# YihangChen-ee/CNC

Measured on AMD Instinct MI355X. Metric: ray-samples/s/GPU (16Lx2^19xF8 grid), higher is better.
Workload: dtype f32; 1 GPU; configs[1]: 800x800 rays/GPU marched (step 5e-3) through a 128^3 ball occupancy, every sample encoded fwd (sign bit plane) + bwd (STE mask) on the binarised 16Lx2^19xF8 hash grid; rays_per_gpu=640000, chunk=1048576, table_rows=6120776, n_features=8, levels=16

## Files before the change

cnc_amd/_lib.py:

```python
from __future__ import annotations

import ctypes as C
import os

import torch

_HERE = os.path.dirname(os.path.abspath(__file__))
LIB_PATH = os.path.join(_HERE, "libcnc_hip.so")
_lib = None

_vp, _u32, _i32, _i64, _f32 = C.c_void_p, C.c_uint32, C.c_int32, C.c_int64, C.c_float


class RaySegments(C.Structure):
    _fields_ = [("vals", _vp), ("chunk_starts", _vp), ("chunk_cnts", _vp), ("ray_indices", _vp),
                ("is_left", _vp), ("is_right", _vp), ("is_valid", _vp)]


class PdfRows(C.Structure):
    _fields_ = [("seg", RaySegments), ("n_rays", _i64), ("n_edges_per_ray", _i64), ("n_edges", _i64)]


class CtxWindow(C.Structure):
    _fields_ = [("pos", _vp * 16), ("cnt", _vp * 16), ("val", _vp * 16), ("p_at", _i64 * 17), ("v_at", _i64 * 17),
# ... 134 lines not shown
    "cnc_rows_scatter": [_vp, _vp, _vp, C.c_uint64, _u32, _vp],
    "cnc_table_adam": [_vp] + [C.c_double] * 6 + [_vp],
    "cnc_ray_window_positions": [_vp] * 10 + [_u32, _vp],
    "cnc_scatter_counted": [_vp, _vp, _vp, _vp, C.c_uint64, _vp],
    "cnc_ctx_compact": [_vp, _vp, _vp, _vp, C.c_uint64, _i32, _vp, _vp, _vp, _vp, _vp],
    "cnc_plane_ring_vertices": [_vp, C.c_uint64, _u32, _u32, C.c_uint64, _vp, _vp, _vp],
    "cnc_bernoulli_bits_partials": [C.c_uint64, _u32],
    "cnc_bernoulli_bits_forward": [_vp, _vp, _vp, C.c_uint64, _u32, _vp, _vp],
    "cnc_bernoulli_bits_backward": [_vp, _vp, _vp, _vp, C.c_uint64, _u32, _vp, _vp, _vp],
    "cnc_segment_weighted_sum_backward": [_vp, _vp, _vp, _vp, _u32, C.c_uint64, _u32, _i32, _vp, _vp],
    "cnc_segment_weighted_sum_gathered_backward": [_vp, _vp, _vp, _vp, _vp, _u32, C.c_uint64, _u32, _i32, _vp, _vp],
}

RESTYPES = {"cnc_grid_encode_backward_binned_workspace": C.c_uint64,
            "cnc_grid_encode_backward_overlapped_workspace": C.c_uint64, "cnc_bernoulli_bits_partials": C.c_uint32,
            "cnc_relu_backward_bias_partials": C.c_uint32, "cnc_occupancy_coarse_words": C.c_uint32}

CNC_FLAG_STE_BINARY = 1
CNC_FLAG_LEVELS_FINEST_FIRST = 2
CNC_FLAG_BIN_LANE_STORES = 4
CNC_FLAG_CELL_MERGE = 8
CNC_FLAG_CELL_CARRY = 16
CNC_FLAG_OWNER_XCD_PAIRS = 32
CNC_FIELD_SH_FP16 = 1
CNC_FIELD_MFMA_F16X3 = 2
CNC_FIELD_TWO_WAVES = 4
CNC_FIELD_WAVES4 = 8
CNC_PACK_TRANSPOSE = 1
CNC_PACK_ZERO_FIRST = 2
CNC_VOLREND_ACCUMULATE = 1
CNC_VOLREND_FINALIZE = 2
ABI_VERSION = 32


def lib() -> C.CDLL:
    global _lib
    if _lib is None:
        if not os.path.exists(LIB_PATH):
            raise RuntimeError(
                f"{LIB_PATH} not found: the HIP extension is required (no CPU fallback). "
                "Build it with `python -m cnc_amd.build`.")
        L = C.CDLL(LIB_PATH)
        for name, argtypes in SIGNATURES.items():
            fn = getattr(L, name)
            fn.argtypes = argtypes
            fn.restype = RESTYPES.get(name, C.c_int)
# ... 50 lines not shown
```

cnc_amd/backends/gridencoder_backend.py:

```python
from __future__ import annotations

import os

import torch

from .. import _lib
from .._lib import check, check_contiguous, check_cuda, ptr, stream

_FLOATING = (torch.float32, torch.float16, torch.float64)


def _check_floating(t, name):
    if t.dtype not in _FLOATING:
        raise RuntimeError(f"{name} must be a floating tensor")


def _check_int(t, name):
    if t.dtype != torch.int32:
        raise RuntimeError(f"{name} must be an int tensor")


def _require_f32(t, name):
    if t.dtype != torch.float32:
        raise RuntimeError(f"{name}: libcnc_hip builds the fp32 path only (got {t.dtype})")
# ... 100 lines not shown
                    ("offsets_list", offsets_list), ("resolutions_list", resolutions_list),
                    ("grad_embeddings", grad_embeddings)])
    _check_floating(grad, "grad")
    _check_floating(inputs, "inputs")
    _check_floating(embeddings, "embeddings")
    _check_int(offsets_list, "offsets_list")
    _check_int(resolutions_list, "resolutions_list")
    _check_floating(grad_embeddings, "grad_embeddings")
    for name, t in (("grad", grad), ("inputs", inputs), ("embeddings", embeddings),
                    ("grad_embeddings", grad_embeddings)):
        _require_f32(t, name)
    if n_features not in (1, 2, 4, 8, 16, 32):
        raise RuntimeError("GridEncoding: n_fearures must be 1, 2, 4, 8, 16 or 32.")
    if num_dim not in (1, 2, 3):
        raise RuntimeError("GridEncoding: num_dim must be 1, 2, 3.")
    if binary_vxl is not None:
        binary_vxl = binary_vxl.contiguous()
    if binned is not None and binned[0] > 0 and binary_vxl is None and min_level_id is None \
            and dy_dx is None and grad_inputs is None:
        n_binned, level_rows = int(binned[0]), int(binned[1])
        L = _lib.lib()
        nbytes = int(L.cnc_grid_encode_backward_binned_workspace(int(N), n_binned, level_rows))
        flags = (_lib.CNC_FLAG_STE_BINARY if ste_binary else 0) | (_lib.CNC_FLAG_BIN_LANE_STORES if _BIN_LANE_STORES else 0) \
            | (_lib.CNC_FLAG_OWNER_XCD_PAIRS if _OWNER_XCD_PAIRS else 0)
        if overlap_streams and _OVERLAP_ENABLED:
            cur = torch.cuda.current_stream(grad.device).cuda_stream
            nbytes = int(L.cnc_grid_encode_backward_overlapped_workspace(int(N), n_binned, level_rows))
            ws = _workspace(grad.device, nbytes, (cur, 0))
            rc = L.cnc_grid_encode_backward_overlapped(
                _plan(grad.device, cur), ptr(grad), ptr(inputs), ptr(embeddings), ptr(offsets_list), ptr(resolutions_list),
                ptr(grad_embeddings), int(N), int(num_dim), int(n_features), int(n_levels), flags, ptr(ste_clip_count),
                int(grad_ld), int(grad_col), n_binned, level_rows, ptr(ws),
                nbytes, stream(grad.device))
            check(rc, "grid_encode_backward_overlapped")
            return
        ws = _workspace(grad.device, nbytes, (torch.cuda.current_stream(grad.device).cuda_stream, 0))
        rc = L.cnc_grid_encode_backward_binned(
            ptr(grad), ptr(inputs), ptr(embeddings), ptr(offsets_list), ptr(resolutions_list),
            ptr(grad_embeddings), int(N), int(num_dim), int(n_features), int(n_levels), flags,
            ptr(ste_clip_count), int(grad_ld), int(grad_col), n_binned, level_rows, ptr(ws), nbytes,
            stream(grad.device))
        check(rc, "grid_encode_backward_binned")
        return
    rc = _lib.lib().cnc_grid_encode_backward(
        ptr(grad), ptr(inputs), ptr(embeddings), ptr(offsets_list), ptr(resolutions_list),
        ptr(grad_embeddings), int(N), int(num_dim), int(n_features), int(n_levels), int(Rb),
        ptr(dy_dx), ptr(grad_inputs), ptr(binary_vxl), ptr(min_level_id),
        (_lib.CNC_FLAG_STE_BINARY if ste_binary else 0)
        | (_lib.CNC_FLAG_LEVELS_FINEST_FIRST if interleave_levels else 0)
        | (_lib.CNC_FLAG_CELL_MERGE if cell_merge else 0)
        | (_lib.CNC_FLAG_CELL_CARRY if cell_merge and cell_carry else 0), ptr(ste_clip_count),
        ptr(_check_sat(occ_sat, binary_vxl)), *_vb(vertex_bits, binary_vxl, 0 if min_level_id is not None else n_levels),
        int(grad_ld), int(grad_col), stream(grad.device))
    check(rc, "grid_encode_backward")


_WORKSPACES = {}
_PLANS = {}
_OVERLAP_ENABLED = os.environ.get("CNC_BWD_OVERLAP", "1") != "0"
_BIN_LANE_STORES = os.environ.get("CNC_BWD_BIN_LANE_STORES", "0") == "1"
_OWNER_XCD_PAIRS = os.environ.get("CNC_BWD_OWNER_XCD_PAIRS", "0") == "1"


def _plan(device, caller_stream):
    import ctypes as C
    key = (device.type, device.index, caller_stream)
    h = _PLANS.get(key)
    if h is None:
        out = C.c_void_p()
        with torch.cuda.device(device):
            check(_lib.lib().cnc_backward_plan_create(C.byref(out)), "backward_plan_create")
        h = _PLANS[key] = out
    return h


def _workspace(device, nbytes, which=0):
    key = (device.type, device.index, which)
    ws = _WORKSPACES.get(key)
    if ws is None or ws.numel() < nbytes:
        ws = torch.empty(nbytes, dtype=torch.uint8, device=device)
        _WORKSPACES[key] = ws
    return ws


# ... 233 lines not shown
```

cnc_amd/csrc/common.hpp:

```cpp
#pragma once

#include <hip/hip_runtime.h>
#include <stdint.h>
#include <stdlib.h>

#include "cnc_hip.h"

namespace cnc {

constexpr int kWave = 64;

__host__ __device__ inline uint32_t div_up(uint32_t a, uint32_t b) { return (a + b - 1) / b; }

struct FeatLayout {
    uint32_t ld;
    uint32_t col;
    uint32_t finest_first = 0;
    uint32_t n_slots = 0;
    const uint32_t* vbits = nullptr;
    const int32_t*  vboff = nullptr;
    uint32_t        nt = 0;
};

__device__ __forceinline__ const uint32_t* vertex_plane(const FeatLayout& lay, uint32_t level)
{
    if (lay.vbits == nullptr) return nullptr;
    const int32_t w = lay.vboff[level];
    return w < 0 ? nullptr : lay.vbits + w;
}

__device__ __forceinline__ size_t feat_index(FeatLayout lay, uint32_t slot, uint32_t N, uint32_t b,
                                             uint32_t F)
{
    return lay.ld ? (size_t)b * lay.ld + lay.col + slot * F : ((size_t)slot * N + b) * F;
}

inline int launch_status()
{
    return hipGetLastError() == hipSuccess ? CNC_OK : CNC_ERR_LAUNCH;
}

template <uint32_t D>
__device__ __forceinline__ uint32_t grid_row(const uint32_t (&q)[D], uint32_t hashmap_size,
                                             uint32_t resolution)
{
    constexpr uint32_t primes[7] = {1u, 2654435761u, 805459861u, 3674653429u,
                                    2097192037u, 1434869437u, 2165219737u};
    uint32_t stride = 1, index = 0;
#pragma unroll
    for (uint32_t d = 0; d < D; d++) {
        if (stride <= hashmap_size) {
            index += q[d] * stride;
            stride *= resolution;
        }
    }
    if (stride > hashmap_size) {
        index = 0;
#pragma unroll
// ... 82 lines not shown
```

cnc_amd/csrc/grid_encode.hip:

```cpp
#include "common.hpp"
#include <cstdlib>

#include "encoder_common.hpp"

namespace cnc {

template <uint32_t D, uint32_t F, bool VXL, bool STE>
__global__ __launch_bounds__(256) void k_grid_encode_fwd(
    const float* __restrict__ inputs, const float* __restrict__ emb,
    const int32_t* __restrict__ offsets, const int32_t* __restrict__ resolutions,
    float* __restrict__ out, uint32_t N, uint32_t Rb, const uint8_t* __restrict__ vxl,
    const int32_t* __restrict__ min_level_id, const int32_t* __restrict__ sat, FeatLayout lay)
{
    constexpr uint32_t V = F < 4 ? F : 4;
    constexpr uint32_t G = F / V;
    constexpr uint32_t C = 1u << D;

    const uint32_t t = blockIdx.x * blockDim.x + threadIdx.x;
    const uint32_t b = t / G;
    const uint32_t h = t % G;
    if (b >= N) return;
    const uint32_t slot = blockIdx.y;
    const uint32_t level = slot + (min_level_id ? (uint32_t)min_level_id[b] : 0u);

// ... 615 lines not shown
    if (!cnt_loc(inputs + (size_t)b * 3, R, F, axis, q, loc)) return;
    const size_t   at = (size_t)grid_row<3>(q, hs, R) * F;
    const uint32_t half = loc / 2;
    const float gv = 1 / out_sum[half + ch];
    const bool  pos = (double)emb[at + ch] > 0.9;
    const float contrib = pos ? gv * grad[loc + ch * 2 + 0] : -gv * grad[loc + ch * 2 + 1];
    unsafeAtomicAdd(grad_emb + at + ch, contrib);
}

struct EncArgs {
    const float*   inputs;
    const float*   emb;
    const int32_t* offsets;
    const int32_t* resolutions;
    float*         out;
    const float*   grad;
    uint32_t       N, L, Rb;
    const uint8_t* vxl;
    const int32_t* mli;
    hipStream_t    stream;
    const uint32_t* clip_count = nullptr;
    const int32_t*  sat = nullptr;
    FeatLayout      lay{0, 0};
};

template <uint32_t D, uint32_t F, bool VXL, bool STE>
static void launch_fwd(const EncArgs& a)
{
    constexpr uint32_t V = F < 4 ? F : 4, G = F / V;
    const dim3 grid(div_up(a.N * G, 256), a.L, 1);
    hipLaunchKernelGGL((k_grid_encode_fwd<D, F, VXL, STE>), grid, dim3(256), 0, a.stream,
                       a.inputs, a.emb, a.offsets, a.resolutions, a.out, a.N, a.Rb, a.vxl, a.mli, a.sat, a.lay);
}

bool launch_bwd_cells(const CellsArgs& a, uint32_t D, uint32_t F, bool ste, hipStream_t s);

void launch_bwd_merge(const float* grad, const float* inputs, const float* emb, const int32_t* offsets,
                      const int32_t* resolutions, float* grad_emb, uint32_t N, uint32_t L,
                      const uint32_t* clip_count, FeatLayout lay, bool ste, hipStream_t s);

template <uint32_t D, uint32_t F, bool VXL, bool STE>
static void launch_bwd(const EncArgs& a)
{
    if constexpr (D == 3 && F == 8 && !VXL) {
        if (a.lay.finest_first && !a.mli && (uint64_t)div_up(a.N, 256) * a.L < (1ull << 31)) {
            launch_bwd_merge(a.grad, a.inputs, a.emb, a.offsets, a.resolutions, a.out, a.N, a.L, a.clip_count,
                             a.lay, STE, a.stream);
            return;
        }
    }
    if constexpr ((1u << D) * F <= 64) {
        const uint64_t blocks = (uint64_t)div_up(a.N, 256) * a.L;
        FeatLayout     lay = a.lay;
        dim3           grid(div_up(a.N, 256), a.L, 1);
        if (a.lay.finest_first && blocks < (1ull << 31)) {
            lay.n_slots = a.L;
            grid = dim3((uint32_t)blocks, 1, 1);
        }
        hipLaunchKernelGGL((k_grid_encode_bwd<D, F, VXL, STE>), grid, dim3(256), 0, a.stream,
                           a.grad, a.inputs, a.emb, a.offsets, a.resolutions, a.out, a.N, a.Rb,
                           a.vxl, a.mli, a.clip_count, a.sat, lay);
    } else {
        constexpr uint32_t V = F < 4 ? F : 4, G = F / V;
        const dim3 grid(div_up(a.N * G, 256), a.L, 1);
        hipLaunchKernelGGL((k_grid_encode_bwd_simple<D, F, VXL, STE>), grid, dim3(256), 0,
                           a.stream, a.grad, a.inputs, a.emb, a.offsets, a.resolutions, a.out, a.N,
                           a.Rb, a.vxl, a.mli, a.clip_count, a.sat, a.lay);
    }
}

// ... 61 lines not shown
                                       const int32_t* offsets, const int32_t* resolutions,
                                       float* outputs, uint32_t N, uint32_t D, uint32_t F,
                                       uint32_t L, uint32_t Rb, float PV, float* dy_dx,
                                       const uint8_t* binary_vxl, const int32_t* min_level_id,
                                       uint32_t flags, const int32_t* occ_sat,
                                       const uint32_t* vertex_bits, const int32_t* vertex_bit_offsets,
                                       uint32_t out_ld, uint32_t out_col, void* stream)
{
    (void)PV;
    if (N == 0 || L == 0) return CNC_OK;
    if (!inputs || !embeddings || !offsets || !resolutions || !outputs) return CNC_ERR_INVALID_VALUE;
    EncArgs a{inputs, embeddings, offsets, resolutions, outputs, nullptr, N, L, Rb,
              binary_vxl, min_level_id, (hipStream_t)stream, nullptr, binary_vxl ? occ_sat : nullptr,
              FeatLayout{out_ld, out_col}};
    if (!layout_ok(a.lay, F, L)) return CNC_ERR_INVALID_VALUE;
    if (binary_vxl && vertex_bits && vertex_bit_offsets) { a.lay.vbits = vertex_bits; a.lay.vboff = vertex_bit_offsets; }
    int rc = dispatch_D<false>(a, D, F, (flags & CNC_FLAG_STE_BINARY) != 0);
    if (rc == CNC_OK && dy_dx)
        rc = launch_dy_dx(inputs, embeddings, offsets, resolutions, dy_dx, N, D, F, L, min_level_id,
                          (flags & CNC_FLAG_STE_BINARY) != 0, (hipStream_t)stream);
    return rc != CNC_OK ? rc : launch_status();
}

extern "C" int cnc_grid_encode_backward(const float* grad, const float* inputs,
                                        const float* embeddings, const int32_t* offsets,
                                        const int32_t* resolutions, float* grad_embeddings,
                                        uint32_t N, uint32_t D, uint32_t F, uint32_t L,
                                        uint32_t Rb, const float* dy_dx, float* grad_inputs,
                                        const uint8_t* binary_vxl, const int32_t* min_level_id,
                                        uint32_t flags, const uint32_t* ste_clip_count,
                                        const int32_t* occ_sat, const uint32_t* vertex_bits,
                                        const int32_t* vertex_bit_offsets, uint32_t grad_ld,
                                        uint32_t grad_col, void* stream)
{
    if ((dy_dx == nullptr) != (grad_inputs == nullptr)) return CNC_ERR_INVALID_VALUE;
    if (N == 0 || L == 0) return CNC_OK;
    if (!grad || !inputs || !embeddings || !offsets || !resolutions || !grad_embeddings)
        return CNC_ERR_INVALID_VALUE;
    EncArgs a{inputs, embeddings, offsets, resolutions, grad_embeddings, grad, N, L, Rb,
              binary_vxl, min_level_id, (hipStream_t)stream, ste_clip_count,
              binary_vxl ? occ_sat : nullptr,
              FeatLayout{grad_ld, grad_col, (flags & CNC_FLAG_LEVELS_FINEST_FIRST) ? 1u : 0u}};
    if (!layout_ok(a.lay, F, L)) return CNC_ERR_INVALID_VALUE;
    if (binary_vxl && vertex_bits && vertex_bit_offsets) { a.lay.vbits = vertex_bits; a.lay.vboff = vertex_bit_offsets; }
    int rc = CNC_OK;
    bool done = false;
    if ((flags & CNC_FLAG_CELL_MERGE) && !dy_dx) {
        const CellsArgs ca{grad, inputs, embeddings, offsets, resolutions, grad_embeddings, binary_vxl, min_level_id,
                           ste_clip_count, a.sat, a.lay, N, L, Rb, (flags & CNC_FLAG_CELL_CARRY) ? 1u : 0u};
        done = launch_bwd_cells(ca, D, F, (flags & CNC_FLAG_STE_BINARY) != 0, (hipStream_t)stream);
    }
    if (!done) rc = dispatch_D<true>(a, D, F, (flags & CNC_FLAG_STE_BINARY) != 0);
    if (rc == CNC_OK && dy_dx)
        rc = launch_input_backward(grad, dy_dx, grad_inputs, N, D, F, L, FeatLayout{grad_ld, grad_col},
                                   (hipStream_t)stream);
    return rc != CNC_OK ? rc : launch_status();
}

#define CNC_F_SWITCH(F, CALL)                         \
    switch (F) {                                      \
    case 1: { constexpr uint32_t FF = 1; CALL; } break;   \
    case 2: { constexpr uint32_t FF = 2; CALL; } break;   \
    case 4: { constexpr uint32_t FF = 4; CALL; } break;   \
    case 8: { constexpr uint32_t FF = 8; CALL; } break;   \
    case 16: { constexpr uint32_t FF = 16; CALL; } break; \
    case 32: { constexpr uint32_t FF = 32; CALL; } break; \
    default: return CNC_ERR_INVALID_VALUE;            \
    }

extern "C" int cnc_cnt_np_embed(const int16_t* inputs, const float* embeddings_clip,
                                float* outputs, uint32_t N, uint32_t resolution, uint32_t F,
                                uint32_t hashmap_size, uint32_t axis, void* stream)
{
    if (N == 0) return CNC_OK;
    if (!inputs || !embeddings_clip || !outputs || axis > 2) return CNC_ERR_INVALID_VALUE;
    CNC_F_SWITCH(F, hipLaunchKernelGGL((k_cnt_np_embed<FF>), dim3(div_up(div_up(N, 8) * 2 * FF, 256)),
                                       dim3(256), 0, (hipStream_t)stream, inputs, embeddings_clip,
                                       outputs, N, resolution, hashmap_size, axis));
    return launch_status();
// ... 152 lines not shown
```

cnc_amd/csrc/grid_encode_binned.hip:

```cpp
#include "common.hpp"
#include "encoder_common.hpp"

namespace cnc {

constexpr uint32_t kSlabLog2 = 8;
constexpr uint32_t kSlab = 1u << kSlabLog2;
constexpr uint32_t kBinSamplesPerThread = 4;
constexpr uint32_t kMaxBins = 4096;
constexpr uint32_t kHeadBytes = 16;

struct Item {
    uint32_t sample;
    float    w0, w1;
    uint32_t rows;
};
static_assert(sizeof(Item) == 16, "Item is read as one dwordx4");

struct BinnedArgs {
    const float*    grad;
    const float*    inputs;
    const float*    emb;
    const int32_t*  offsets;
    const int32_t*  resolutions;
    float*          grad_emb;
// ... 515 lines not shown
extern "C" uint64_t cnc_grid_encode_backward_binned_workspace(uint32_t N, uint32_t n_binned,
                                                              uint32_t level_rows)
{
    if (n_binned == 0 || level_rows == 0) return 0;
    const uint64_t bins = div_up(level_rows, kSlab);
    return (uint64_t)n_binned * bins * (kHeadBytes + (uint64_t)default_cap(N, (uint32_t)bins) * sizeof(Item));
}

extern "C" int cnc_grid_encode_backward_binned(const float* grad, const float* inputs,
                                               const float* embeddings, const int32_t* offsets,
                                               const int32_t* resolutions, float* grad_embeddings,
                                               uint32_t N, uint32_t D, uint32_t F, uint32_t L,
                                               uint32_t flags, const uint32_t* ste_clip_count,
                                               uint32_t grad_ld, uint32_t grad_col,
                                               uint32_t n_binned, uint32_t level_rows,
                                               void* workspace, uint64_t workspace_bytes,
                                               void* stream)
{
    if (N == 0 || L == 0) return CNC_OK;
    if (!grad || !inputs || !embeddings || !offsets || !resolutions || !grad_embeddings)
        return CNC_ERR_INVALID_VALUE;
    if (n_binned > L) return CNC_ERR_INVALID_VALUE;
    if (L - n_binned > 0) {
        const int rc = cnc_grid_encode_backward(grad, inputs, embeddings, offsets, resolutions,
                                                grad_embeddings, N, D, F, L - n_binned, 0, nullptr,
                                                nullptr, nullptr, nullptr,
                                                flags | CNC_FLAG_LEVELS_FINEST_FIRST, ste_clip_count,
                                                nullptr, nullptr, nullptr, grad_ld, grad_col, stream);
        if (rc != CNC_OK) return rc;
    }
    if (n_binned == 0) return CNC_OK;
    if (D != 3 || !(F == 2 || F == 4 || F == 8)) return CNC_ERR_UNSUPPORTED;
    if (grad_ld != 0) {
        const uint32_t V = F < 4 ? F : 4;
        if (grad_col + L * F > grad_ld || grad_ld % V || grad_col % V) return CNC_ERR_INVALID_VALUE;
    } else if (grad_col != 0) {
        return CNC_ERR_INVALID_VALUE;
    }
    const uint32_t bins = div_up(level_rows, kSlab);
    if (bins == 0 || bins > kMaxBins || !workspace) return CNC_ERR_INVALID_VALUE;
    const uint64_t heads = (uint64_t)n_binned * bins;
    if ((uintptr_t)workspace % 16 != 0) return CNC_ERR_INVALID_VALUE;
    if (workspace_bytes < heads * (kHeadBytes + 64 * sizeof(Item))) return CNC_ERR_INVALID_VALUE;
    uint64_t cap = (workspace_bytes - heads * kHeadBytes) / (heads * sizeof(Item));
    if (cap > 0x0FFFFFFFull) cap = 0x0FFFFFFFull;

    hipStream_t s = (hipStream_t)stream;
    uint32_t*   ws = (uint32_t*)workspace;
    if (hipMemsetAsync(ws, 0, heads * 4, s) != hipSuccess) return CNC_ERR_LAUNCH;
    const uint32_t part = owner_part(N, bins, cap), parts = div_up((uint32_t)cap, part);
    const uint32_t n_pairs = (flags & CNC_FLAG_OWNER_XCD_PAIRS) ? n_binned / 2 : 0;
// ... 14 lines not shown
```

cnc_amd/csrc/grid_encode_merge.hip:

```cpp
#include <cstdlib>

#include "common.hpp"
#include "encoder_common.hpp"

namespace cnc {

typedef float f32x4 __attribute__((ext_vector_type(4)));

template <bool STE, uint32_t MB>
__global__ __launch_bounds__(MB) void k_grid_encode_bwd_merge(
    const float* __restrict__ grad, const float* __restrict__ inputs, const float* __restrict__ emb,
    const int32_t* __restrict__ offsets, const int32_t* __restrict__ resolutions,
    float* __restrict__ grad_emb, uint32_t N, const uint32_t* __restrict__ clip_count, FeatLayout lay)
{
    constexpr uint32_t kMB = MB;
    constexpr uint32_t kMW = kMB / 64;
    constexpr uint32_t kMSlots = kMB <= 512 ? 1024 : 2048;
    constexpr uint32_t D = 3, F = 8, C = 8, END = 0x7FFu;
    static_assert(kMB <= 1024, "run records pack start (10 bits) / end (11) / next (11)");
    __shared__ __attribute__((aligned(16))) float s_w4[kMB][4];
    __shared__ float    s_g[kMB][F];
    __shared__ __attribute__((aligned(16))) uint4 s_u[kMB];
    uint64_t* const s_key = reinterpret_cast<uint64_t*>(s_u);
    uint32_t* const h_slot = reinterpret_cast<uint32_t*>(s_u) + 2 * kMB;
    static_assert(kMSlots * 4 <= kMB * 8, "hash table fits the second half of s_u");
    __shared__ uint16_t s_run_start[kMB + 1];
    __shared__ uint32_t l_head[kMB];
    __shared__ uint32_t s_run_rec[kMB];
    __shared__ uint32_t s_wave_heads[kMW], s_wave_claims[kMW];

    const uint32_t tid = threadIdx.x, lane = tid & 63, wave = tid >> 6;
    const bool     mask_on = STE && (clip_count == nullptr || *clip_count != 0);
    const uint32_t n_slots = lay.n_slots;
    const uint32_t chunk = blockIdx.x / n_slots;
    const uint32_t slot = n_slots - 1 - blockIdx.x % n_slots;
    const uint32_t b = chunk * kMB + tid;
    const uint32_t off = (uint32_t)offsets[slot];
    const uint32_t hs = (uint32_t)offsets[slot + 1] - off;
    const uint32_t R = (uint32_t)resolutions[slot];

    for (uint32_t i = tid; i < kMSlots; i += kMB) h_slot[i] = 0;
    l_head[tid] = END;

    uint64_t key = ~0ull;
    uint32_t validmask = 0;
    {
        float    x[D];
        if (b < N && load_point<D>(inputs, b, x)) {
            Corners<D, false> c;
            c.setup(x, R, hs, 0, nullptr);
            key = (uint64_t)c.cell[0] | (uint64_t)c.cell[1] << 16 | (uint64_t)c.cell[2] << 32;
            if (R > kCellKeyMaxRes) key = ~0ull;
#pragma unroll
            for (uint32_t i = 0; i < C; i++) validmask |= (c.valid[i] ? 1u : 0u) << i;
            *reinterpret_cast<float4*>(s_w4[tid]) = make_float4(c.frac[0], c.frac[1], c.frac[2], c.wn_re);
            const float* gp = grad + feat_index(lay, slot, N, b, F);
            float        g0[4], g1[4];
            load_vec<4>(gp, g0);
            load_vec<4>(gp + 4, g1);
#pragma unroll
            for (uint32_t j = 0; j < 4; j++) {
                s_g[tid][j] = g0[j];
                s_g[tid][4 + j] = g1[j];
// ... 160 lines not shown
                for (uint32_t d = 0; d < D; d++) {
                    const bool     bit = (i >> d) & 1u;
                    const uint32_t q = bit ? min(cell[d] + 1, R - 1) : cell[d];
                    wi *= bit ? frac[d] : 1 - frac[d];
                    border |= (q == 0) | (q == R - 1);
                }
                valid |= (border ? 0u : 1u) << i;
                wn += border ? 0.0f : wi;
            }
            if (wn == 0) wn = 1e-9f;
            const float* gp = grad + feat_index(lay, slot, N, b, F);
            float        g[F];
            bool         nonzero = false;
#pragma unroll
            for (uint32_t k = 0; k < F; k++) {
                g[k] = gp[k];
                nonzero |= g[k] != 0.0f;
            }
            if (nonzero) scatter_point<D, F>(cell, frac, valid, 1.0f / wn, off, hs, R, g, emb, grad_emb, mask_on);
        }
    }
}

void launch_bwd_merge(const float* grad, const float* inputs, const float* emb, const int32_t* offsets,
                      const int32_t* resolutions, float* grad_emb, uint32_t N, uint32_t L,
                      const uint32_t* clip_count, FeatLayout lay, bool ste, hipStream_t s)
{
    lay.n_slots = L;
    const bool small = (uint64_t)div_up(N, 1024u) * L < 4096u;
    if (small) {
        const dim3 grid(div_up(N, 512u) * L);
        if (ste) hipLaunchKernelGGL((k_grid_encode_bwd_merge<true, 512>), grid, dim3(512), 0, s, grad, inputs, emb, offsets, resolutions, grad_emb, N, clip_count, lay);
        else hipLaunchKernelGGL((k_grid_encode_bwd_merge<false, 512>), grid, dim3(512), 0, s, grad, inputs, emb, offsets, resolutions, grad_emb, N, clip_count, lay);
    } else {
        const dim3 grid(div_up(N, 1024u) * L);
        if (ste) hipLaunchKernelGGL((k_grid_encode_bwd_merge<true, 1024>), grid, dim3(1024), 0, s, grad, inputs, emb, offsets, resolutions, grad_emb, N, clip_count, lay);
        else hipLaunchKernelGGL((k_grid_encode_bwd_merge<false, 1024>), grid, dim3(1024), 0, s, grad, inputs, emb, offsets, resolutions, grad_emb, N, clip_count, lay);
    }
    const dim3 wide(div_up(N, 256u) < 16u ? div_up(N, 256u) : 16u, L);
    if (ste) hipLaunchKernelGGL((k_grid_encode_bwd_wide<true>), wide, dim3(256), 0, s, grad, inputs, emb, offsets, resolutions, grad_emb, N, clip_count, lay);
    else hipLaunchKernelGGL((k_grid_encode_bwd_wide<false>), wide, dim3(256), 0, s, grad, inputs, emb, offsets, resolutions, grad_emb, N, clip_count, lay);
}

}
```

cnc_amd/csrc/grid_encode_overlap.hip:

```cpp
#include <hip/hip_runtime.h>

#include <cstdlib>
#include <new>

#include "cnc_hip.h"

struct cnc_backward_plan {
    hipStream_t side[2];
    hipEvent_t  fork;
    hipEvent_t  join[2];
    int         device;
    int         group_split;
};

namespace {
constexpr uint32_t kMinOverlapPoints = 1u << 16;
constexpr uint64_t kAlign = 256;

inline uint64_t round_up(uint64_t v) { return (v + kAlign - 1) / kAlign * kAlign; }

inline int split_groups(uint32_t n_binned, int group_split, uint32_t first[2], uint32_t count[2])
{
    if (group_split > 0 && (uint32_t)group_split < n_binned) {
        count[0] = (uint32_t)group_split; count[1] = n_binned - count[0];
        first[0] = 0; first[1] = count[0];
        return 2;
    }
    first[0] = 0; count[0] = n_binned;
// ... 23 lines not shown
    return CNC_OK;
}

extern "C" int cnc_backward_plan_destroy(cnc_backward_plan* p)
{
    if (!p) return CNC_OK;
    for (int i = 0; i < 2; ++i) {
        (void)hipStreamSynchronize(p->side[i]);
        (void)hipStreamDestroy(p->side[i]);
        (void)hipEventDestroy(p->join[i]);
    }
    (void)hipEventDestroy(p->fork);
    delete p;
    return CNC_OK;
}

extern "C" uint64_t cnc_grid_encode_backward_overlapped_workspace(uint32_t N, uint32_t n_binned, uint32_t level_rows)
{
    uint64_t total = 0;
    if (n_binned >= 2)
        total = round_up(cnc_grid_encode_backward_binned_workspace(N, 1, level_rows))
                + round_up(cnc_grid_encode_backward_binned_workspace(N, n_binned - 1, level_rows));
    const uint64_t serial = cnc_grid_encode_backward_binned_workspace(N, n_binned, level_rows);
    return total > serial ? total : serial;
}

extern "C" int cnc_grid_encode_backward_overlapped(cnc_backward_plan* plan, const float* grad, const float* inputs,
                                                   const float* embeddings, const int32_t* offsets,
                                                   const int32_t* resolutions, float* grad_embeddings,
                                                   uint32_t N, uint32_t D, uint32_t F, uint32_t L, uint32_t flags,
                                                   const uint32_t* ste_clip_count, uint32_t grad_ld, uint32_t grad_col,
                                                   uint32_t n_binned, uint32_t level_rows,
                                                   void* workspace, uint64_t workspace_bytes, void* stream)
{
    if (N == 0 || L == 0) return CNC_OK;
    if (n_binned > L) return CNC_ERR_INVALID_VALUE;
    const uint32_t coarse = L - n_binned;
    if (!plan || coarse == 0 || n_binned == 0 || N < kMinOverlapPoints)
        return cnc_grid_encode_backward_binned(grad, inputs, embeddings, offsets, resolutions, grad_embeddings, N, D, F, L,
                                               flags, ste_clip_count, grad_ld, grad_col, n_binned, level_rows, workspace,
                                               workspace_bytes, stream);
    if (!grad || !inputs || !embeddings || !offsets || !resolutions || !grad_embeddings || !workspace)
        return CNC_ERR_INVALID_VALUE;
    if ((uintptr_t)workspace % 16 != 0) return CNC_ERR_INVALID_VALUE;
    hipStream_t s = (hipStream_t)stream;
    uint32_t first[2], count[2];
    const int groups = split_groups(n_binned, plan->group_split, first, count);
    if (hipEventRecord(plan->fork, s) != hipSuccess) return CNC_ERR_LAUNCH;
    int rc = CNC_OK;
    uint64_t used = 0;
    for (int g = 0; g < groups; ++g) {
        const uint32_t l0 = coarse + first[g];
        uint64_t share = g + 1 < groups ? workspace_bytes * count[g] / n_binned / kAlign * kAlign : workspace_bytes - used;
        char* ws = (char*)workspace + used;
        used += share;
        const float*   g_grad = grad_ld == 0 ? grad + (uint64_t)l0 * N * F : grad;
        const uint32_t g_col = grad_ld == 0 ? grad_col : grad_col + l0 * F;
        if (hipStreamWaitEvent(plan->side[g], plan->fork, 0) != hipSuccess) return CNC_ERR_LAUNCH;
        const int rg = cnc_grid_encode_backward_binned(g_grad, inputs, embeddings, offsets + l0, resolutions + l0,
                                                       grad_embeddings, N, D, F, count[g], flags, ste_clip_count, grad_ld,
                                                       g_col, count[g], level_rows, ws, share, plan->side[g]);
        if (rg != CNC_OK && rc == CNC_OK) rc = rg;
        if (hipEventRecord(plan->join[g], plan->side[g]) != hipSuccess) return CNC_ERR_LAUNCH;
    }
    const int rc0 = cnc_grid_encode_backward(grad, inputs, embeddings, offsets, resolutions, grad_embeddings, N, D, F, coarse,
                                             0, nullptr, nullptr, nullptr, nullptr, flags | CNC_FLAG_LEVELS_FINEST_FIRST,
                                             ste_clip_count, nullptr, nullptr, nullptr, grad_ld, grad_col, stream);
    for (int g = 0; g < groups; ++g)
        if (hipStreamWaitEvent(s, plan->join[g], 0) != hipSuccess) return CNC_ERR_LAUNCH;
    return rc0 != CNC_OK ? rc0 : rc;
}
```

include/cnc_hip.h:

```cpp
#ifndef CNC_HIP_H
#define CNC_HIP_H

#include <stdint.h>

#ifdef __cplusplus
extern "C" {
#endif

#define CNC_OK                 0
#define CNC_ERR_INVALID_VALUE -1
#define CNC_ERR_UNSUPPORTED   -2
#define CNC_ERR_LAUNCH        -3

#define CNC_F32 0

#define CNC_FLAG_NONE        0u
#define CNC_FLAG_STE_BINARY  1u
#define CNC_FLAG_LEVELS_FINEST_FIRST 2u
#define CNC_FLAG_BIN_LANE_STORES 4u
#define CNC_FLAG_OWNER_XCD_PAIRS 32u

#define CNC_FLAG_CELL_MERGE 8u
#define CNC_FLAG_CELL_CARRY 16u

const char* cnc_error_string(int code);
int         cnc_abi_version(void);


int cnc_grid_encode_forward(const float* inputs, const float* embeddings,
                            const int32_t* offsets, const int32_t* resolutions,
                            float* outputs,
                            uint32_t N, uint32_t D, uint32_t F, uint32_t L,
                            uint32_t Rb, float PV,
                            float* dy_dx, const uint8_t* binary_vxl, const int32_t* min_level_id,
                            uint32_t flags, const int32_t* occ_sat,
                            const uint32_t* vertex_bits, const int32_t* vertex_bit_offsets,
                            uint32_t out_ld, uint32_t out_col, void* stream);

uint64_t cnc_grid_vertex_bits_words(uint32_t D, uint32_t R);
int cnc_grid_vertex_bits(const int32_t* occ_sat, uint32_t D, uint32_t Rb, uint32_t R, uint32_t* words, void* stream);

int cnc_grid_encode_backward(const float* grad, const float* inputs, const float* embeddings,
                             const int32_t* offsets, const int32_t* resolutions,
// ... 480 lines not shown
```

Before: 866.9 million ray-samples/s.

## Reorder merge-kernel sample tiles by ray depth for spatially coherent backward scatter

Adds a pre-pass kernel that, per 8192-sample window, estimates the ray direction, computes a depth key for each 8-sample segment and bitonic-sorts the segments so that each 1024-thread merge block covers spatially nearby samples across rays. For levels at or above a minimum resolution, the backward merge kernel then gathers samples through this tile order. The goal is more duplicate-vertex merging in shared memory and fewer global atomics on fine levels. In exchange it adds an extra kernel launch and a scratch buffer carved from the workspace, and gather indirection costs coalescing of grad and input loads.

New measurement: 881.8 million ray-samples/s, median of 6. 1.02x the previous value.

```diff
diff --git a/cnc_amd/_lib.py b/cnc_amd/_lib.py
--- a/cnc_amd/_lib.py
+++ b/cnc_amd/_lib.py
@@ -180,6 +180,7 @@
 CNC_FLAG_CELL_MERGE = 8
 CNC_FLAG_CELL_CARRY = 16
 CNC_FLAG_OWNER_XCD_PAIRS = 32
+CNC_FLAG_MERGE_CONSECUTIVE = 64
 CNC_FIELD_SH_FP16 = 1
 CNC_FIELD_MFMA_F16X3 = 2
 CNC_FIELD_TWO_WAVES = 4
diff --git a/cnc_amd/backends/gridencoder_backend.py b/cnc_amd/backends/gridencoder_backend.py
--- a/cnc_amd/backends/gridencoder_backend.py
+++ b/cnc_amd/backends/gridencoder_backend.py
@@ -146,7 +146,7 @@
         L = _lib.lib()
         nbytes = int(L.cnc_grid_encode_backward_binned_workspace(int(N), n_binned, level_rows))
         flags = (_lib.CNC_FLAG_STE_BINARY if ste_binary else 0) | (_lib.CNC_FLAG_BIN_LANE_STORES if _BIN_LANE_STORES else 0) \
-            | (_lib.CNC_FLAG_OWNER_XCD_PAIRS if _OWNER_XCD_PAIRS else 0)
+            | (_lib.CNC_FLAG_OWNER_XCD_PAIRS if _OWNER_XCD_PAIRS else 0) | (0 if _MERGE_TILES else _lib.CNC_FLAG_MERGE_CONSECUTIVE)
         if overlap_streams and _OVERLAP_ENABLED:
             cur = torch.cuda.current_stream(grad.device).cuda_stream
             nbytes = int(L.cnc_grid_encode_backward_overlapped_workspace(int(N), n_binned, level_rows))
@@ -172,6 +172,7 @@
         ptr(dy_dx), ptr(grad_inputs), ptr(binary_vxl), ptr(min_level_id),
         (_lib.CNC_FLAG_STE_BINARY if ste_binary else 0)
         | (_lib.CNC_FLAG_LEVELS_FINEST_FIRST if interleave_levels else 0)
+        | (0 if _MERGE_TILES else _lib.CNC_FLAG_MERGE_CONSECUTIVE)
         | (_lib.CNC_FLAG_CELL_MERGE if cell_merge else 0)
         | (_lib.CNC_FLAG_CELL_CARRY if cell_merge and cell_carry else 0), ptr(ste_clip_count),
         ptr(_check_sat(occ_sat, binary_vxl)), *_vb(vertex_bits, binary_vxl, 0 if min_level_id is not None else n_levels),
@@ -184,6 +185,7 @@
 _OVERLAP_ENABLED = os.environ.get("CNC_BWD_OVERLAP", "1") != "0"
 _BIN_LANE_STORES = os.environ.get("CNC_BWD_BIN_LANE_STORES", "0") == "1"
 _OWNER_XCD_PAIRS = os.environ.get("CNC_BWD_OWNER_XCD_PAIRS", "0") == "1"
+_MERGE_TILES = os.environ.get("CNC_BWD_MERGE_TILES", "1") != "0"
 
 
 def _plan(device, caller_stream):
diff --git a/cnc_amd/csrc/common.hpp b/cnc_amd/csrc/common.hpp
--- a/cnc_amd/csrc/common.hpp
+++ b/cnc_amd/csrc/common.hpp
@@ -34,6 +34,15 @@
 {
     return lay.ld ? (size_t)b * lay.ld + lay.col + slot * F : ((size_t)slot * N + b) * F;
 }
+
+int grid_encode_backward_with_scratch(const float* grad, const float* inputs, const float* embeddings, const int32_t* offsets,
+                                      const int32_t* resolutions, float* grad_embeddings, uint32_t N, uint32_t D, uint32_t F,
+                                      uint32_t L, uint32_t Rb, const float* dy_dx, float* grad_inputs,
+                                      const uint8_t* binary_vxl, const int32_t* min_level_id, uint32_t flags,
+                                      const uint32_t* ste_clip_count, const int32_t* occ_sat, const uint32_t* vertex_bits,
+                                      const int32_t* vertex_bit_offsets, uint32_t grad_ld, uint32_t grad_col, void* stream,
+                                      uint16_t* tile_order);
+uint64_t merge_tile_order_bytes(uint32_t N);
 
 inline int launch_status()
 {
diff --git a/cnc_amd/csrc/grid_encode.hip b/cnc_amd/csrc/grid_encode.hip
--- a/cnc_amd/csrc/grid_encode.hip
+++ b/cnc_amd/csrc/grid_encode.hip
@@ -661,6 +661,8 @@
     const uint32_t* clip_count = nullptr;
     const int32_t*  sat = nullptr;
     FeatLayout      lay{0, 0};
+    bool            merge_consecutive = false;
+    uint16_t*       tile_order = nullptr;
 };
 
 template <uint32_t D, uint32_t F, bool VXL, bool STE>
@@ -676,7 +678,8 @@
 
 void launch_bwd_merge(const float* grad, const float* inputs, const float* emb, const int32_t* offsets,
                       const int32_t* resolutions, float* grad_emb, uint32_t N, uint32_t L,
-                      const uint32_t* clip_count, FeatLayout lay, bool ste, hipStream_t s);
+                      const uint32_t* clip_count, FeatLayout lay, bool ste, bool consecutive, uint16_t* tile_order,
+                      hipStream_t s);
 
 template <uint32_t D, uint32_t F, bool VXL, bool STE>
 static void launch_bwd(const EncArgs& a)
@@ -684,7 +687,7 @@
     if constexpr (D == 3 && F == 8 && !VXL) {
         if (a.lay.finest_first && !a.mli && (uint64_t)div_up(a.N, 256) * a.L < (1ull << 31)) {
             launch_bwd_merge(a.grad, a.inputs, a.emb, a.offsets, a.resolutions, a.out, a.N, a.L, a.clip_count,
-                             a.lay, STE, a.stream);
+                             a.lay, STE, a.merge_consecutive, a.tile_order, a.stream);
             return;
         }
     }
@@ -792,6 +795,43 @@
     return rc != CNC_OK ? rc : launch_status();
 }
 
+int cnc::grid_encode_backward_with_scratch(const float* grad, const float* inputs,
+                                           const float* embeddings, const int32_t* offsets,
+                                           const int32_t* resolutions, float* grad_embeddings,
+                                           uint32_t N, uint32_t D, uint32_t F, uint32_t L,
+                                           uint32_t Rb, const float* dy_dx, float* grad_inputs,
+                                           const uint8_t* binary_vxl, const int32_t* min_level_id,
+                                           uint32_t flags, const uint32_t* ste_clip_count,
+                                           const int32_t* occ_sat, const uint32_t* vertex_bits,
+                                           const int32_t* vertex_bit_offsets, uint32_t grad_ld,
+                                           uint32_t grad_col, void* stream, uint16_t* tile_order)
+{
+    if ((dy_dx == nullptr) != (grad_inputs == nullptr)) return CNC_ERR_INVALID_VALUE;
+    if (N == 0 || L == 0) return CNC_OK;
+    if (!grad || !inputs || !embeddings || !offsets || !resolutions || !grad_embeddings)
+        return CNC_ERR_INVALID_VALUE;
+    EncArgs a{inputs, embeddings, offsets, resolutions, grad_embeddings, grad, N, L, Rb,
+              binary_vxl, min_level_id, (hipStream_t)stream, ste_clip_count,
+              binary_vxl ? occ_sat : nullptr,
+              FeatLayout{grad_ld, grad_col, (flags & CNC_FLAG_LEVELS_FINEST_FIRST) ? 1u : 0u}};
+    if (!layout_ok(a.lay, F, L)) return CNC_ERR_INVALID_VALUE;
+    a.merge_consecutive = (flags & CNC_FLAG_MERGE_CONSECUTIVE) != 0;
+    a.tile_order = tile_order;
+    if (binary_vxl && vertex_bits && vertex_bit_offsets) { a.lay.vbits = vertex_bits; a.lay.vboff = vertex_bit_offsets; }
+    int rc = CNC_OK;
+    bool done = false;
+    if ((flags & CNC_FLAG_CELL_MERGE) && !dy_dx) {
+        const CellsArgs ca{grad, inputs, embeddings, offsets, resolutions, grad_embeddings, binary_vxl, min_level_id,
+                           ste_clip_count, a.sat, a.lay, N, L, Rb, (flags & CNC_FLAG_CELL_CARRY) ? 1u : 0u};
+        done = launch_bwd_cells(ca, D, F, (flags & CNC_FLAG_STE_BINARY) != 0, (hipStream_t)stream);
+    }
+    if (!done) rc = dispatch_D<true>(a, D, F, (flags & CNC_FLAG_STE_BINARY) != 0);
+    if (rc == CNC_OK && dy_dx)
+        rc = launch_input_backward(grad, dy_dx, grad_inputs, N, D, F, L, FeatLayout{grad_ld, grad_col},
+                                   (hipStream_t)stream);
+    return rc != CNC_OK ? rc : launch_status();
+}
+
 extern "C" int cnc_grid_encode_backward(const float* grad, const float* inputs,
                                         const float* embeddings, const int32_t* offsets,
                                         const int32_t* resolutions, float* grad_embeddings,
@@ -803,28 +843,9 @@
                                         const int32_t* vertex_bit_offsets, uint32_t grad_ld,
                                         uint32_t grad_col, void* stream)
 {
-    if ((dy_dx == nullptr) != (grad_inputs == nullptr)) return CNC_ERR_INVALID_VALUE;
-    if (N == 0 || L == 0) return CNC_OK;
-    if (!grad || !inputs || !embeddings || !offsets || !resolutions || !grad_embeddings)
-        return CNC_ERR_INVALID_VALUE;
-    EncArgs a{inputs, embeddings, offsets, resolutions, grad_embeddings, grad, N, L, Rb,
-              binary_vxl, min_level_id, (hipStream_t)stream, ste_clip_count,
-              binary_vxl ? occ_sat : nullptr,
-              FeatLayout{grad_ld, grad_col, (flags & CNC_FLAG_LEVELS_FINEST_FIRST) ? 1u : 0u}};
-    if (!layout_ok(a.lay, F, L)) return CNC_ERR_INVALID_VALUE;
-    if (binary_vxl && vertex_bits && vertex_bit_offsets) { a.lay.vbits = vertex_bits; a.lay.vboff = vertex_bit_offsets; }
-    int rc = CNC_OK;
-    bool done = false;
-    if ((flags & CNC_FLAG_CELL_MERGE) && !dy_dx) {
-        const CellsArgs ca{grad, inputs, embeddings, offsets, resolutions, grad_embeddings, binary_vxl, min_level_id,
-                           ste_clip_count, a.sat, a.lay, N, L, Rb, (flags & CNC_FLAG_CELL_CARRY) ? 1u : 0u};
-        done = launch_bwd_cells(ca, D, F, (flags & CNC_FLAG_STE_BINARY) != 0, (hipStream_t)stream);
-    }
-    if (!done) rc = dispatch_D<true>(a, D, F, (flags & CNC_FLAG_STE_BINARY) != 0);
-    if (rc == CNC_OK && dy_dx)
-        rc = launch_input_backward(grad, dy_dx, grad_inputs, N, D, F, L, FeatLayout{grad_ld, grad_col},
-                                   (hipStream_t)stream);
-    return rc != CNC_OK ? rc : launch_status();
+    return grid_encode_backward_with_scratch(grad, inputs, embeddings, offsets, resolutions, grad_embeddings, N, D, F, L, Rb,
+                                             dy_dx, grad_inputs, binary_vxl, min_level_id, flags, ste_clip_count, occ_sat,
+                                             vertex_bits, vertex_bit_offsets, grad_ld, grad_col, stream, nullptr);
 }
 
 #define CNC_F_SWITCH(F, CALL)                         \
diff --git a/cnc_amd/csrc/grid_encode_binned.hip b/cnc_amd/csrc/grid_encode_binned.hip
--- a/cnc_amd/csrc/grid_encode_binned.hip
+++ b/cnc_amd/csrc/grid_encode_binned.hip
@@ -561,11 +561,18 @@
         return CNC_ERR_INVALID_VALUE;
     if (n_binned > L) return CNC_ERR_INVALID_VALUE;
     if (L - n_binned > 0) {
-        const int rc = cnc_grid_encode_backward(grad, inputs, embeddings, offsets, resolutions,
-                                                grad_embeddings, N, D, F, L - n_binned, 0, nullptr,
-                                                nullptr, nullptr, nullptr,
-                                                flags | CNC_FLAG_LEVELS_FINEST_FIRST, ste_clip_count,
-                                                nullptr, nullptr, nullptr, grad_ld, grad_col, stream);
+        uint16_t*      tile_order = nullptr;
+        const uint64_t order_bytes = merge_tile_order_bytes(N);
+        const uint64_t bins_bytes = (cnc_grid_encode_backward_binned_workspace(N, n_binned, level_rows) + 255) / 256 * 256;
+        if (workspace && (uintptr_t)workspace % 16 == 0 && workspace_bytes >= bins_bytes + order_bytes) {
+            workspace_bytes = (workspace_bytes - order_bytes) / 256 * 256;
+            tile_order = reinterpret_cast<uint16_t*>((char*)workspace + workspace_bytes);
+        }
+        const int rc = grid_encode_backward_with_scratch(grad, inputs, embeddings, offsets, resolutions,
+                                                         grad_embeddings, N, D, F, L - n_binned, 0, nullptr,
+                                                         nullptr, nullptr, nullptr,
+                                                         flags | CNC_FLAG_LEVELS_FINEST_FIRST, ste_clip_count,
+                                                         nullptr, nullptr, nullptr, grad_ld, grad_col, stream, tile_order);
         if (rc != CNC_OK) return rc;
     }
     if (n_binned == 0) return CNC_OK;
diff --git a/cnc_amd/csrc/grid_encode_merge.hip b/cnc_amd/csrc/grid_encode_merge.hip
--- a/cnc_amd/csrc/grid_encode_merge.hip
+++ b/cnc_amd/csrc/grid_encode_merge.hip
@@ -7,11 +7,105 @@
 
 typedef float f32x4 __attribute__((ext_vector_type(4)));
 
-template <bool STE, uint32_t MB>
+#ifndef CNC_MERGE_TILE_WINDOW
+#define CNC_MERGE_TILE_WINDOW 8192
+#endif
+#ifndef CNC_MERGE_TILE_SEGMENT
+#define CNC_MERGE_TILE_SEGMENT 8
+#endif
+constexpr uint32_t kMergeTileWindow = CNC_MERGE_TILE_WINDOW, kMergeTileSegment = CNC_MERGE_TILE_SEGMENT;
+#ifndef CNC_MERGE_TILE_MIN_RES
+#define CNC_MERGE_TILE_MIN_RES 52
+#endif
+constexpr uint32_t kMergeTileMinRes = CNC_MERGE_TILE_MIN_RES;
+
+template <uint32_t TW, uint32_t TS>
+__global__ __launch_bounds__(1024) void k_merge_tile_order(const float* __restrict__ inputs, uint32_t N,
+                                                           uint16_t* __restrict__ order)
+{
+    constexpr uint32_t MB = 1024;
+    __shared__ uint32_t s_sort[2 * MB], s_cnt[MB / 64];
+    const uint32_t base = blockIdx.x * TW;
+    constexpr uint32_t kSegs = TW / TS, kTiles = TW / MB;
+    constexpr uint32_t kPastEnd = 0x3FFFFFu, kUnusable = 0x3FFFFEu;
+    static_assert(MB == 1024 && kSegs <= MB && kSegs * TS == TW && kTiles * MB == TW, "one segment per thread, 10 index bits");
+    static_assert(TS >= 1 && TS <= 16 && (TS & (TS - 1)) == 0 && (kTiles & (kTiles - 1)) == 0 && kTiles <= 16,
+                  "a tile is at least one wave of segments");
+    const uint32_t tid = threadIdx.x, lane = tid & 63, wave = tid >> 6;
+    const uint32_t n_in = min(N - base, TW), n_seg = div_up(n_in, TS);
+    float ax[3] = {0.0f, 0.0f, 0.0f};
+    if (n_in >= 2) {
+        float cand[3][3], len[3];
+#pragma unroll
+        for (uint32_t k = 0; k < 3; k++) {
+            const size_t a = (size_t)base + min(k * 11u, n_in - 2);
+#pragma unroll
+            for (uint32_t d = 0; d < 3; d++) cand[k][d] = inputs[(a + 1) * 3 + d] - inputs[a * 3 + d];
+            len[k] = (cand[k][0] * cand[k][0] + cand[k][1] * cand[k][1]) + cand[k][2] * cand[k][2];
+        }
+        const bool m0 = len[0] <= len[1] ? (len[1] > len[2] && len[0] > len[2]) : len[0] <= len[2];
+        const bool m2 = len[0] <= len[1] ? (len[1] > len[2] && len[0] <= len[2]) : (len[0] > len[2] && len[1] <= len[2]);
+#pragma unroll
+        for (uint32_t d = 0; d < 3; d++) ax[d] = m0 ? cand[0][d] : m2 ? cand[2][d] : cand[1][d];
+    }
+    uint32_t q = kPastEnd;
+    if (tid < n_seg) {
+        const size_t s = (size_t)base + min(tid * TS + TS / 2, n_in - 1);
+        const float  x0 = inputs[s * 3], x1 = inputs[s * 3 + 1], x2 = inputs[s * 3 + 2];
+        const float  dep = (x0 * ax[0] + x1 * ax[1]) + x2 * ax[2];
+        const bool   usable = x0 >= 0 && x0 <= 1 && x1 >= 0 && x1 <= 1 && x2 >= 0 && x2 <= 1 && dep == dep;
+        uint32_t     u = __float_as_uint(dep);
+        u ^= (u >> 31) ? 0xFFFFFFFFu : 0x80000000u;
+        q = usable ? min(u >> 10, kUnusable - 1) : kUnusable;
+    }
+    const uint32_t qp = (uint32_t)__shfl_up((int)q, 1);
+    const uint64_t db = __ballot(lane != 0 && q < qp && qp < kUnusable);
+    if (lane == 0) s_cnt[wave] = (uint32_t)__popcll(db);
+    uint32_t key = q << 10 | tid;
+#pragma unroll
+    for (uint32_t k = 2; k <= 64; k <<= 1) {
+        uint32_t o = (uint32_t)__shfl_xor((int)key, (int)(k - 1));
+        key = (lane & (k >> 1)) == 0 ? min(key, o) : max(key, o);
+#pragma unroll
+        for (uint32_t s = k >> 2; s >= 1; s >>= 1) {
+            o = (uint32_t)__shfl_xor((int)key, (int)s);
+            key = (lane & s) == 0 ? min(key, o) : max(key, o);
+        }
+    }
+    __syncthreads();
+    uint32_t n_rays = 1;
+#pragma unroll
+    for (uint32_t w = 0; w < MB / 64; w++) n_rays += s_cnt[w];
+    const uint32_t have = n_rays * kSegs * 5u, want = n_seg * 32u * 7u;
+    uint32_t       n_sub = have < want ? 1u : have < 2 * want ? 2u : have < 4 * want ? 4u : have < 8 * want ? 8u : 16u;
+    n_sub = min(n_sub, kTiles);
+    const uint32_t sub_segs = kSegs / n_sub;
+    uint32_t p = 0;
+    auto cross = [&](uint32_t mask, uint32_t bit) {
+        s_sort[p * MB + tid] = key;
+        __syncthreads();
+        const uint32_t o = s_sort[p * MB + (tid ^ mask)];
+        key = (tid & bit) == 0 ? min(key, o) : max(key, o);
+        p ^= 1;
+    };
+    for (uint32_t k = 128; k <= sub_segs; k <<= 1) {
+        cross(k - 1, k >> 1);
+        for (uint32_t s = k >> 2; s >= 64; s >>= 1) cross(s, s);
+#pragma unroll
+        for (uint32_t s = 32; s >= 1; s >>= 1) {
+            const uint32_t o = (uint32_t)__shfl_xor((int)key, (int)s);
+            key = (lane & s) == 0 ? min(key, o) : max(key, o);
+        }
+    }
+    if (tid < kSegs) order[(size_t)blockIdx.x * kSegs + tid] = (uint16_t)(key & (MB - 1));
+}
+
+template <bool STE, uint32_t MB, uint32_t TW, uint32_t TS>
 __global__ __launch_bounds__(MB) void k_grid_encode_bwd_merge(
     const float* __restrict__ grad, const float* __restrict__ inputs, const float* __restrict__ emb,
     const int32_t* __restrict__ offsets, const int32_t* __restrict__ resolutions,
-    float* __restrict__ grad_emb, uint32_t N, const uint32_t* __restrict__ clip_count, FeatLayout lay)
+    float* __restrict__ grad_emb, uint32_t N, const uint32_t* __restrict__ clip_count, FeatLayout lay,
+    const uint16_t* __restrict__ tile_order)
 {
     constexpr uint32_t kMB = MB;
     constexpr uint32_t kMW = kMB / 64;
@@ -34,11 +128,18 @@
     const uint32_t n_slots = lay.n_slots;
     const uint32_t chunk = blockIdx.x / n_slots;
     const uint32_t slot = n_slots - 1 - blockIdx.x % n_slots;
-    const uint32_t b = chunk * kMB + tid;
+    uint32_t       b = chunk * kMB + tid;
     const uint32_t off = (uint32_t)offsets[slot];
     const uint32_t hs = (uint32_t)offsets[slot + 1] - off;
     const uint32_t R = (uint32_t)resolutions[slot];
 
+    if constexpr (TW != 0) {
+        if (R >= kMergeTileMinRes) {
+            constexpr uint32_t kTiles = TW / kMB, kSegs = TW / TS;
+            const uint32_t win = chunk / kTiles, at = chunk % kTiles * (kMB / TS) + tid / TS;
+            b = win * TW + (uint32_t)tile_order[(size_t)win * kSegs + at] * TS + tid % TS;
+        }
+    }
     for (uint32_t i = tid; i < kMSlots; i += kMB) h_slot[i] = 0;
     l_head[tid] = END;
 
@@ -245,21 +346,34 @@
     }
 }
 
+uint64_t merge_tile_order_bytes(uint32_t N)
+{
+    return ((uint64_t)div_up(N, kMergeTileWindow) * (kMergeTileWindow / kMergeTileSegment) * 2 + 255) / 256 * 256;
+}
+
 void launch_bwd_merge(const float* grad, const float* inputs, const float* emb, const int32_t* offsets,
                       const int32_t* resolutions, float* grad_emb, uint32_t N, uint32_t L,
-                      const uint32_t* clip_count, FeatLayout lay, bool ste, hipStream_t s)
+                      const uint32_t* clip_count, FeatLayout lay, bool ste, bool consecutive, uint16_t* tile_order,
+                      hipStream_t s)
 {
     lay.n_slots = L;
     const bool small = (uint64_t)div_up(N, 1024u) * L < 4096u;
+#define CNC_MERGE_GO(ST, MBS, W, S)                                                                                \
+    hipLaunchKernelGGL((k_grid_encode_bwd_merge<ST, MBS, W, S>), dim3(div_up(N, MBS) * L), dim3(MBS), 0, s, grad, inputs, \
+                       emb, offsets, resolutions, grad_emb, N, clip_count, lay, tile_order)
     if (small) {
-        const dim3 grid(div_up(N, 512u) * L);
-        if (ste) hipLaunchKernelGGL((k_grid_encode_bwd_merge<true, 512>), grid, dim3(512), 0, s, grad, inputs, emb, offsets, resolutions, grad_emb, N, clip_count, lay);
-        else hipLaunchKernelGGL((k_grid_encode_bwd_merge<false, 512>), grid, dim3(512), 0, s, grad, inputs, emb, offsets, resolutions, grad_emb, N, clip_count, lay);
+        if (ste) CNC_MERGE_GO(true, 512u, 0u, 0u);
+        else CNC_MERGE_GO(false, 512u, 0u, 0u);
+    } else if (consecutive || tile_order == nullptr) {
+        if (ste) CNC_MERGE_GO(true, 1024u, 0u, 0u);
+        else CNC_MERGE_GO(false, 1024u, 0u, 0u);
     } else {
-        const dim3 grid(div_up(N, 1024u) * L);
-        if (ste) hipLaunchKernelGGL((k_grid_encode_bwd_merge<true, 1024>), grid, dim3(1024), 0, s, grad, inputs, emb, offsets, resolutions, grad_emb, N, clip_count, lay);
-        else hipLaunchKernelGGL((k_grid_encode_bwd_merge<false, 1024>), grid, dim3(1024), 0, s, grad, inputs, emb, offsets, resolutions, grad_emb, N, clip_count, lay);
-    }
+        hipLaunchKernelGGL((k_merge_tile_order<kMergeTileWindow, kMergeTileSegment>), dim3(div_up(N, kMergeTileWindow)),
+                           dim3(1024), 0, s, inputs, N, tile_order);
+        if (ste) CNC_MERGE_GO(true, 1024u, kMergeTileWindow, kMergeTileSegment);
+        else CNC_MERGE_GO(false, 1024u, kMergeTileWindow, kMergeTileSegment);
+    }
+#undef CNC_MERGE_GO
     const dim3 wide(div_up(N, 256u) < 16u ? div_up(N, 256u) : 16u, L);
     if (ste) hipLaunchKernelGGL((k_grid_encode_bwd_wide<true>), wide, dim3(256), 0, s, grad, inputs, emb, offsets, resolutions, grad_emb, N, clip_count, lay);
     else hipLaunchKernelGGL((k_grid_encode_bwd_wide<false>), wide, dim3(256), 0, s, grad, inputs, emb, offsets, resolutions, grad_emb, N, clip_count, lay);
diff --git a/cnc_amd/csrc/grid_encode_overlap.hip b/cnc_amd/csrc/grid_encode_overlap.hip
--- a/cnc_amd/csrc/grid_encode_overlap.hip
+++ b/cnc_amd/csrc/grid_encode_overlap.hip
@@ -4,6 +4,7 @@
 #include <new>
 
 #include "cnc_hip.h"
+#include "common.hpp"
 
 struct cnc_backward_plan {
     hipStream_t side[2];
@@ -73,7 +74,7 @@
         total = round_up(cnc_grid_encode_backward_binned_workspace(N, 1, level_rows))
                 + round_up(cnc_grid_encode_backward_binned_workspace(N, n_binned - 1, level_rows));
     const uint64_t serial = cnc_grid_encode_backward_binned_workspace(N, n_binned, level_rows);
-    return total > serial ? total : serial;
+    return round_up(total > serial ? total : serial) + cnc::merge_tile_order_bytes(N);
 }
 
 extern "C" int cnc_grid_encode_backward_overlapped(cnc_backward_plan* plan, const float* grad, const float* inputs,
@@ -95,6 +96,11 @@
         return CNC_ERR_INVALID_VALUE;
     if ((uintptr_t)workspace % 16 != 0) return CNC_ERR_INVALID_VALUE;
     hipStream_t s = (hipStream_t)stream;
+    uint16_t* tile_order = nullptr;
+    if (workspace_bytes >= cnc_grid_encode_backward_overlapped_workspace(N, n_binned, level_rows)) {
+        workspace_bytes = (workspace_bytes - cnc::merge_tile_order_bytes(N)) / kAlign * kAlign;
+        tile_order = reinterpret_cast<uint16_t*>((char*)workspace + workspace_bytes);
+    }
     uint32_t first[2], count[2];
     const int groups = split_groups(n_binned, plan->group_split, first, count);
     if (hipEventRecord(plan->fork, s) != hipSuccess) return CNC_ERR_LAUNCH;
@@ -114,9 +120,10 @@
         if (rg != CNC_OK && rc == CNC_OK) rc = rg;
         if (hipEventRecord(plan->join[g], plan->side[g]) != hipSuccess) return CNC_ERR_LAUNCH;
     }
-    const int rc0 = cnc_grid_encode_backward(grad, inputs, embeddings, offsets, resolutions, grad_embeddings, N, D, F, coarse,
-                                             0, nullptr, nullptr, nullptr, nullptr, flags | CNC_FLAG_LEVELS_FINEST_FIRST,
-                                             ste_clip_count, nullptr, nullptr, nullptr, grad_ld, grad_col, stream);
+    const int rc0 = cnc::grid_encode_backward_with_scratch(grad, inputs, embeddings, offsets, resolutions, grad_embeddings, N, D, F,
+                                                      coarse, 0, nullptr, nullptr, nullptr, nullptr,
+                                                      flags | CNC_FLAG_LEVELS_FINEST_FIRST, ste_clip_count, nullptr, nullptr,
+                                                      nullptr, grad_ld, grad_col, stream, tile_order);
     for (int g = 0; g < groups; ++g)
         if (hipStreamWaitEvent(s, plan->join[g], 0) != hipSuccess) return CNC_ERR_LAUNCH;
     return rc0 != CNC_OK ? rc0 : rc;
diff --git a/include/cnc_hip.h b/include/cnc_hip.h
--- a/include/cnc_hip.h
+++ b/include/cnc_hip.h
@@ -19,6 +19,8 @@
 #define CNC_FLAG_LEVELS_FINEST_FIRST 2u
 #define CNC_FLAG_BIN_LANE_STORES 4u
 #define CNC_FLAG_OWNER_XCD_PAIRS 32u
+
+#define CNC_FLAG_MERGE_CONSECUTIVE 64u
 
 #define CNC_FLAG_CELL_MERGE 8u
 #define CNC_FLAG_CELL_CARRY 16u
```
